# julius-speech/julius

Hardware: AMD Instinct MI355X
Metric: frames_x_states_scored_per_sec (higher is better)
Workload: dtype f32; 1 GPU; C2 = configs[1]: triphone GMM outprob only, S=3000 M=16 D=39, step = 12 launches x 64000 frames; frames_per_launch=64000, parallelism=utterance-sharded x1, kernel=gmm_tile<D=39,FPL=2,NS=16,ring> grid=24000 nsb=16

## Files before the change

julius_amd/csrc/gmm_outprob.hip:

```cpp
#include "gmm_dev.h"
#include "gmm_host.h"

namespace {
using namespace jamd;

constexpr int kWaves = 4;

template <int D, int FPL, int NS, bool HAS_NULL>
__global__ void __launch_bounds__(64 * kWaves)
gmm_tile_kernel(const float *__restrict__ rec, const int *__restrict__ st_off,
                const float *__restrict__ frames, const float *__restrict__ tbl,
                float *__restrict__ out, int T, int S, int nsb, int nfb, int nstb,
                float addmin_f) {
  static_assert(FPL % 2 == 0, "frames are processed as packed pairs");
  constexpr int REC = ((2 * D + 2) + 3) & ~3;
  constexpr int FPW = 64 * FPL;
  constexpr int NP = FPL / 2;
  __shared__ float tile[kWaves][FPW][NS + 1];

  int fb, sb;
  if (!decode_block(nfb, nstb, fb, sb)) return;
  const int lane = threadIdx.x & 63;
  const int wave = threadIdx.x >> 6;
  const int t0 = (fb * kWaves + wave) * FPW;
  if (t0 >= T) return;

  f2 v[NP][D];
#pragma unroll
  for (int p = 0; p < NP; p++) load_frames<D>(v[p], nullptr, frames, t0 + p * 128, T, D, lane);

#if defined(__HIP_DEVICE_COMPILE__) && !defined(__GFX9__)
#error "gmm_tile: the raw buffer descriptor below is the gfx9 (CDNA) format; this library is written for gfx950 only"
#endif
  const __amdgpu_buffer_rsrc_t tbl_rsrc = __builtin_amdgcn_make_buffer_rsrc((void *)tbl, 0, 4 * (JAMD_TBLSIZE + 1), 0x00020000);
  const int s_begin = sb * nsb;
  const int s_end = min(S, s_begin + nsb);
  for (int sg = s_begin; sg < s_end; sg += NS) {
    const int ns = min(NS, s_end - sg);
    for (int si = 0; si < ns; si++) {
      const int e0 = st_off[sg + si], e1 = st_off[sg + si + 1];
      f2 y2[NP], tv2[NP];
#pragma unroll
      for (int p = 0; p < NP; p++) { y2[p] = f2{JAMD_LOG_ZERO, JAMD_LOG_ZERO}; tv2[p] = f2{0.0f, 0.0f}; }
      for (int e = e1 - 1; e >= e0; e--) {
        const float *__restrict__ r = rec + (size_t)e * REC;
        const float gc = r[2 * D], lw = r[2 * D + 1];
        f2 acc[NP];
#pragma unroll
        for (int p = 0; p < NP; p++) acc[p] = f2{gc, gc};
#pragma unroll
        for (int d = 0; d < D; d++) {
          const float mu = r[d], iv = r[D + d];
          const f2 mu2 = {mu, mu}, iv2 = {iv, iv};
#pragma unroll
          for (int p = 0; p < NP; p++) {
            f2 x = v[p][d] - mu2;
            x = x * x;
            x = x * iv2;
            acc[p] = acc[p] + x;
          }
        }
        const bool nulld = HAS_NULL && (gc != gc);
        const float naddmin = -addmin_f;
#pragma unroll
        for (int p = 0; p < NP; p++) {
          f2 s2 = acc[p] * f2{-0.5f, -0.5f};
          if (nulld) s2 = f2{JAMD_LOG_ZERO, JAMD_LOG_ZERO};
          s2 = s2 + f2{lw, lw};
          __builtin_amdgcn_sched_barrier(0);
          const f2 yy = y2[p] + tv2[p];
          const f2 hi = {__builtin_fmaxf(s2.x, yy.x), __builtin_fmaxf(s2.y, yy.y)};
          const f2 df = s2 - yy;
          const float a0 = __builtin_fabsf(df.x), a1 = __builtin_fabsf(df.y);
          unsigned o0 = ((unsigned)((double)a0 * JAMD_TMAG + 0.5)) << 2, o1 = ((unsigned)((double)a1 * JAMD_TMAG + 0.5)) << 2;
          o0 = (a0 <= naddmin) ? o0 : 4u * (unsigned)JAMD_TBLSIZE;
          o1 = (a1 <= naddmin) ? o1 : 4u * (unsigned)JAMD_TBLSIZE;
          tv2[p] = f2{__builtin_bit_cast(float, __builtin_amdgcn_raw_buffer_load_b32(tbl_rsrc, (int)o0, 0, 0)),
                      __builtin_bit_cast(float, __builtin_amdgcn_raw_buffer_load_b32(tbl_rsrc, (int)o1, 0, 0))};
          y2[p] = hi;
        }
      }
#pragma unroll
      for (int k = 0; k < FPL; k++) {
        const f2 fin = y2[k / 2] + tv2[k / 2];
        tile[wave][k * 64 + lane][si] = finish_state((k & 1) ? fin.y : fin.x);
      }
    }
    wave_sync();
    constexpr int RPI = 64 / NS;
    const int col = lane % NS, rsub = lane / NS;
#pragma unroll 4
    for (int it = 0; it < FPW / RPI; it++) {
      const int rr = it * RPI + rsub;
      const int t = t0 + rr;
      if (t < T && col < ns) out[(size_t)t * S + sg + col] = tile[wave][rr][col];
    }
    wave_release();
  }
}

typedef float f16v __attribute__((ext_vector_type(16)));
constexpr int kRingRec = 80;

template <int BYTE_OFF>
__device__ __forceinline__ void ring_load(f16v &home, const float *chunks) {
  __builtin_amdgcn_sched_barrier(0);
  asm volatile("s_load_dwordx16 %0, %1, %2" : "=s"(home) : "s"(chunks), "i"(BYTE_OFF));
  __builtin_amdgcn_sched_barrier(0);
}
__device__ __forceinline__ void ring_wait(f16v &h0, f16v &h1, f16v &h2) {
  __builtin_amdgcn_sched_barrier(0);
  asm volatile("s_waitcnt lgkmcnt(0)" : "+s"(h0), "+s"(h1), "+s"(h2));
  __builtin_amdgcn_sched_barrier(0);
}
template <int N, int MU0, int IV0>
__device__ __forceinline__ void ring_chunk(f2 &acc, const f2 *v, const f16v &h) {
  f2 x[N], q[N], w[N];
#pragma unroll
  for (int i = 0; i < N + 3; i++) {
    if (i < N) { const float mu = h[MU0 + i]; x[i] = v[i] - f2{mu, mu}; }
    if (i >= 1 && i - 1 < N) q[i - 1] = x[i - 1] * x[i - 1];
    if (i >= 2 && i - 2 < N) { const float iv = h[IV0 + i - 2]; w[i - 2] = q[i - 2] * f2{iv, iv}; }
    if (i >= 3) acc = acc + w[i - 3];
    __builtin_amdgcn_sched_barrier(0);
  }
}

template <int NS, bool HAS_NULL>
__global__ void __launch_bounds__(64 * kWaves)
gmm_tile_ring_kernel(const float *__restrict__ ring, const int *__restrict__ st_off,
                     const float *__restrict__ frames, const float *__restrict__ tbl,
                     float *__restrict__ out, int T, int S, int nsb, int nfb, int nstb,
                     float addmin_f) {
  constexpr int D = 39, FPL = 2;
  constexpr int FPW = 64 * FPL;
  __shared__ float tile[kWaves][FPW][NS + 1];

  int fb, sb;
  if (!decode_block(nfb, nstb, fb, sb)) return;
  const int lane = threadIdx.x & 63;
  const int wave = threadIdx.x >> 6;
  const int t0 = (fb * kWaves + wave) * FPW;
  if (t0 >= T) return;

  f2 v[D];
  load_frames<D>(v, nullptr, frames, t0, T, D, lane);

  const __amdgpu_buffer_rsrc_t tbl_rsrc = __builtin_amdgcn_make_buffer_rsrc((void *)tbl, 0, 4 * (JAMD_TBLSIZE + 1), 0x00020000);
  const float naddmin = -addmin_f;
  const int s_begin = sb * nsb;
  const int s_end = min(S, s_begin + nsb);
  f16v h0, h1, h2;
  int held = -1;
  for (int sg = s_begin; sg < s_end; sg += NS) {
    const int ns = min(NS, s_end - sg);
    for (int si = 0; si < ns; si++) {
      const int s = sg + si;
      const int e0 = st_off[s], e1 = st_off[s + 1];
      const int e_over = (s + 1 < s_end ? st_off[s + 2] : e1) - 1;
      f2 y2 = {JAMD_LOG_ZERO, JAMD_LOG_ZERO}, tv2 = {0.0f, 0.0f};
      if (e1 > e0 && held != e1 - 1) {
        const float *r = ring + (size_t)(e1 - 1) * kRingRec;
        ring_load<0>(h0, r);
        ring_load<64>(h1, r);
        ring_load<128>(h2, r);
        ring_wait(h0, h1, h2);
      }
      for (int e = e1 - 1; e >= e0; e--) {
        const float *r = ring + (size_t)e * kRingRec;
        const float *rn = ring + (size_t)(e > e0 ? e - 1 : e_over) * kRingRec;
        const float gc = h0[0], lw = h0[1];
        const bool nulld = HAS_NULL && (gc != gc);
        f2 acc = {gc, gc};
        ring_chunk<7, 2, 9>(acc, v, h0);
        ring_load<192>(h0, r);
        ring_chunk<8, 0, 8>(acc, v + 7, h1);
        ring_load<256>(h1, r);
        ring_chunk<8, 0, 8>(acc, v + 15, h2);
        ring_wait(h0, h1, h2);
        ring_chunk<8, 0, 8>(acc, v + 23, h0);
        ring_load<0>(h0, rn);
        ring_load<128>(h2, rn);
        ring_chunk<8, 0, 8>(acc, v + 31, h1);
        ring_load<64>(h1, rn);
        {
          f2 s2 = acc * f2{-0.5f, -0.5f};
          if (nulld) s2 = f2{JAMD_LOG_ZERO, JAMD_LOG_ZERO};
          s2 = s2 + f2{lw, lw};
          __builtin_amdgcn_sched_barrier(0);
          const f2 yy = y2 + tv2;
          const f2 hi = {__builtin_fmaxf(s2.x, yy.x), __builtin_fmaxf(s2.y, yy.y)};
          const f2 df = s2 - yy;
          const float a0 = __builtin_fabsf(df.x), a1 = __builtin_fabsf(df.y);
          unsigned o0 = ((unsigned)((double)a0 * JAMD_TMAG + 0.5)) << 2, o1 = ((unsigned)((double)a1 * JAMD_TMAG + 0.5)) << 2;
          o0 = (a0 <= naddmin) ? o0 : 4u * (unsigned)JAMD_TBLSIZE;
          o1 = (a1 <= naddmin) ? o1 : 4u * (unsigned)JAMD_TBLSIZE;
          tv2 = f2{__builtin_bit_cast(float, __builtin_amdgcn_raw_buffer_load_b32(tbl_rsrc, (int)o0, 0, 0)),
                   __builtin_bit_cast(float, __builtin_amdgcn_raw_buffer_load_b32(tbl_rsrc, (int)o1, 0, 0))};
          y2 = hi;
        }
        ring_wait(h0, h1, h2);
      }
      if (e1 > e0) held = e_over;
      const f2 fin = y2 + tv2;
      tile[wave][lane][si] = finish_state(fin.x);
      tile[wave][64 + lane][si] = finish_state(fin.y);
    }
    store_tile<NS, FPW>(tile[wave], out, t0, T, S, sg, ns, lane);
  }
}

template <int FPL, int NS>
__global__ void __launch_bounds__(64 * kWaves)
gmm_tile_generic_kernel(const float *__restrict__ rec, const int *__restrict__ st_off,
                        const float *__restrict__ frames, const float *__restrict__ tbl,
                        float *__restrict__ out, int T, int S, int D, int REC, int nsb, int nfb,
                        int nstb, float addmin_f) {
  static_assert(FPL == 2, "load_frames / gauss_pair hold one packed pair of frames per lane");
  constexpr int FPW = 64 * FPL;
  __shared__ float tile[kWaves][FPW][NS + 1];
  extern __shared__ __align__(16) float dyn[];

  int fb, sb;
  if (!decode_block(nfb, nstb, fb, sb)) return;
  const int lane = threadIdx.x & 63;
  const int wave = threadIdx.x >> 6;
  const int t0 = (fb * kWaves + wave) * FPW;
  if (t0 >= T) return;
  float *vt = dyn + (size_t)wave * D * FPW;
  load_frames<0>(nullptr, vt, frames, t0, T, D, lane);

  const int s_begin = sb * nsb;
  const int s_end = min(S, s_begin + nsb);
  for (int sg = s_begin; sg < s_end; sg += NS) {
    const int ns = min(NS, s_end - sg);
    for (int si = 0; si < ns; si++) {
      const int e0 = st_off[sg + si], e1 = st_off[sg + si + 1];
      float y0 = JAMD_LOG_ZERO, y1 = JAMD_LOG_ZERO;
      for (int e = e1 - 1; e >= e0; e--) {
        const float *__restrict__ r = rec + (size_t)e * REC;
        const float lw = r[2 * D + 1];
        const f2 g = gauss_pair<0>(nullptr, vt, lane, D, r);
        y0 = addlog_step(y0, g.x + lw, tbl, addmin_f);
        y1 = addlog_step(y1, g.y + lw, tbl, addmin_f);
      }
      tile[wave][lane][si] = finish_state(y0);
      tile[wave][64 + lane][si] = finish_state(y1);
    }
    store_tile<NS, FPW>(tile[wave], out, t0, T, S, sg, ns, lane);
  }
}

template <int D, int FPL, int NS>
int launch_tile(jamd_gmm *g, const float *frames, int T, float *out, hipStream_t st) {
  constexpr int FPB = kWaves * 64 * FPL;
  const int nfb = (T + FPB - 1) / FPB;
  const int nsb = NS;
  const int nstb = (g->S + nsb - 1) / nsb;
  const int grid = xcd_grid(nstb, nfb);
  if constexpr (D == 39 && FPL == 2) {
    if (g->has_null)
      hipLaunchKernelGGL((gmm_tile_ring_kernel<NS, true>), dim3(grid), dim3(64 * kWaves), 0, st,
                         g->d_rec_ring, g->d_st_off_plain, frames, g->eng->d_addlog, out, T, g->S, nsb, nfb,
                         nstb, g->eng->addmin_f);
    else
      hipLaunchKernelGGL((gmm_tile_ring_kernel<NS, false>), dim3(grid), dim3(64 * kWaves), 0, st,
                         g->d_rec_ring, g->d_st_off_plain, frames, g->eng->d_addlog, out, T, g->S, nsb, nfb,
                         nstb, g->eng->addmin_f);
    snprintf(g->last_kernel, sizeof(g->last_kernel), "gmm_tile<D=%d,FPL=%d,NS=%d,ring> grid=%d nsb=%d", D, FPL, NS, grid, nsb);
  } else {
    if (g->has_null)
      hipLaunchKernelGGL((gmm_tile_kernel<D, FPL, NS, true>), dim3(grid), dim3(64 * kWaves), 0, st,
                         g->d_rec, g->d_st_off_plain, frames, g->eng->d_addlog, out, T, g->S, nsb, nfb,
                         nstb, g->eng->addmin_f);
    else
      hipLaunchKernelGGL((gmm_tile_kernel<D, FPL, NS, false>), dim3(grid), dim3(64 * kWaves), 0, st,
                         g->d_rec, g->d_st_off_plain, frames, g->eng->d_addlog, out, T, g->S, nsb, nfb,
                         nstb, g->eng->addmin_f);
    snprintf(g->last_kernel, sizeof(g->last_kernel), "gmm_tile<D=%d,FPL=%d,NS=%d> grid=%d nsb=%d", D, FPL, NS, grid, nsb);
  }
  return JAMD_OK;
}

template <int FPL, int NS>
int launch_tile_generic(jamd_gmm *g, const float *frames, int T, float *out, hipStream_t st) {
  constexpr int FPB = kWaves * 64 * FPL;
  const int nfb = (T + FPB - 1) / FPB;
  const int nsb = NS;
  const int nstb = (g->S + nsb - 1) / nsb;
  const int grid = xcd_grid(nstb, nfb);
  const size_t dyn = sizeof(float) * kWaves * g->D * 64 * FPL;
  const int rc = jamd_reserve_dyn_lds((const void *)gmm_tile_generic_kernel<FPL, NS>, dyn, "GMM outprob");
  if (rc != JAMD_OK) return rc;
  hipLaunchKernelGGL((gmm_tile_generic_kernel<FPL, NS>), dim3(grid), dim3(64 * kWaves), dyn, st,
                     g->d_rec, g->d_st_off_plain, frames, g->eng->d_addlog, out, T, g->S, g->D, g->rec,
                     nsb, nfb, nstb, g->eng->addmin_f);
  snprintf(g->last_kernel, sizeof(g->last_kernel), "gmm_tile_generic<FPL=%d,NS=%d> D=%d grid=%d",
           FPL, NS, g->D, grid);
  return JAMD_OK;
}

constexpr int kNarrowT = 256;
constexpr int kNarrowFB = 8;
template <int D, bool HAS_NULL>
__global__ void __launch_bounds__(64)
gmm_narrow_dens_kernel(const float *__restrict__ rec, const float *__restrict__ frames, float *__restrict__ dens, int T, int E,
                       int nfb, int neb) {
  constexpr int REC = (2 * D + 2 + 3) & ~3;
  int fbk, ebk;
  if (!decode_block(nfb, neb, fbk, ebk)) return;
  const int e = ebk * 64 + threadIdx.x;
  const float4 *__restrict__ r4 = reinterpret_cast<const float4 *>(rec + (size_t)(e < E ? e : E - 1) * REC);
  float r[REC];
#pragma unroll
  for (int q = 0; q < REC / 4; q++) { const float4 v = r4[q]; r[4 * q] = v.x; r[4 * q + 1] = v.y; r[4 * q + 2] = v.z; r[4 * q + 3] = v.w; }
  const float gc = r[2 * D], lw = r[2 * D + 1];
  const bool nulld = HAS_NULL && (gc != gc);
  const int t_end = min(T, (fbk + 1) * kNarrowFB);
  for (int t = fbk * kNarrowFB; t < t_end; t += 2) {
    const float *__restrict__ fa = frames + (size_t)t * D;
    const float *__restrict__ fb = frames + (size_t)(t + 1 < T ? t + 1 : t) * D;
    f2 acc = {gc, gc};
#pragma unroll
    for (int d = 0; d < D; d++) {
      f2 x = f2{fa[d], fb[d]} - f2{r[d], r[d]};
      x = x * x;
      x = x * f2{r[D + d], r[D + d]};
      acc = acc + x;
    }
    f2 s2 = acc * f2{-0.5f, -0.5f};
    if (nulld) s2 = f2{JAMD_LOG_ZERO, JAMD_LOG_ZERO};
    s2 = s2 + f2{lw, lw};
    if (e < E) {
      dens[(size_t)t * E + e] = s2.x;
      if (t + 1 < T) dens[(size_t)(t + 1) * E + e] = s2.y;
    }
  }
}

__global__ void __launch_bounds__(256)
gmm_narrow_lse_kernel(const float *__restrict__ dens, const int *__restrict__ st_off, const float *__restrict__ tbl,
                      float *__restrict__ out, int T, int S, int E, float addmin_f) {
  const int i = blockIdx.x * 256 + threadIdx.x;
  if (i >= T * S) return;
  const int t = i / S, s = i - t * S;
  const int e0 = st_off[s], e1 = st_off[s + 1];
  const float *__restrict__ dr = dens + (size_t)t * E;
  float y = JAMD_LOG_ZERO;
  int e = e1 - 1;
  for (; e - 7 >= e0; e -= 8) {
    float v[8];
#pragma unroll
    for (int q = 0; q < 8; q++) v[q] = dr[e - q];
#pragma unroll
    for (int q = 0; q < 8; q++) y = addlog_step(y, v[q], tbl, addmin_f);
  }
  for (; e >= e0; e--) y = addlog_step(y, dr[e], tbl, addmin_f);
  out[(size_t)t * S + s] = finish_state(y);
}

template <int D>
int launch_narrow(jamd_gmm *g, const float *frames, int T, float *out, hipStream_t st) {
  const int E = g->E_plain;
  int rc = jamd_grow(&g->d_narrow, &g->narrow_cap, sizeof(float) * (size_t)kNarrowT * (size_t)E);
  if (rc != JAMD_OK) return rc;
  const int grid = (E + 63) / 64;
  const int nfb = (T + kNarrowFB - 1) / kNarrowFB;
  const dim3 gr(xcd_grid(grid, nfb));
  if (g->has_null) hipLaunchKernelGGL((gmm_narrow_dens_kernel<D, true>), gr, dim3(64), 0, st, g->d_rec, frames, g->d_narrow, T, E, nfb, grid);
  else hipLaunchKernelGGL((gmm_narrow_dens_kernel<D, false>), gr, dim3(64), 0, st, g->d_rec, frames, g->d_narrow, T, E, nfb, grid);
  hipLaunchKernelGGL(gmm_narrow_lse_kernel, dim3((T * g->S + 255) / 256), dim3(256), 0, st, g->d_narrow, g->d_st_off_plain,
                     g->eng->d_addlog, out, T, g->S, E, g->eng->addmin_f);
  snprintf(g->last_kernel, sizeof(g->last_kernel), "gmm_narrow<D=%d> grid=%d + lse", D, grid);
  return JAMD_OK;
}

constexpr int kDensChunk = 1024;
__global__ void __launch_bounds__(64)
gmm_dens_kernel(const float *__restrict__ rec, const float *__restrict__ frames, float *__restrict__ out,
                int T, int E, int D, int REC) {
  extern __shared__ float xs[];
  float (*tile)[17] = reinterpret_cast<float (*)[17]>(xs + (size_t)D * 64);
  const int lane = threadIdx.x;
  const int t0 = blockIdx.x * 64, e_begin = blockIdx.y * kDensChunk;
  const int e_end = min(E, e_begin + kDensChunk);
  {
    int t = t0 + lane; if (t > T - 1) t = T - 1;
    const float *f = frames + (size_t)t * D;
    for (int d = 0; d < D; d++) xs[d * 64 + lane] = f[d];
  }
  wave_sync();
  for (int e0 = e_begin; e0 < e_end; e0 += 16) {
    const int ne = min(16, e_end - e0);
    for (int g = 0; g < ne; g++) {
      const float *__restrict__ r = rec + (size_t)(e0 + g) * REC;
      const float gc = r[2 * D];
      float acc = gc;
      for (int d = 0; d < D; d++) {
        float x = xs[d * 64 + lane] - r[d];
        x = x * x;
        x = x * r[D + d];
        acc = acc + x;
      }
      float sc = acc * -0.5f;
      if (gc != gc) sc = JAMD_LOG_ZERO;
      tile[lane][g] = sc;
    }
    wave_sync();
    const int col = lane & 15, rsub = lane >> 4;
    for (int it = 0; it < 16; it++) {
      const int rr = it * 4 + rsub, t = t0 + rr;
      if (t < T && col < ne) out[(size_t)t * E + e0 + col] = tile[rr][col];
    }
    wave_release();
  }
}

}


int jamd_gmm_launch_plain(jamd_gmm *g, const float *frames, int T, float *out, hipStream_t st) {
  const bool narrow = T <= kNarrowT && g->E_plain > 0;
  return dispatch_veclen(g->D, [&](auto dt) {
    constexpr int D = decltype(dt)::value;
    if constexpr (D == 0) return launch_tile_generic<2, 16>(g, frames, T, out, st);
    else return narrow ? launch_narrow<D>(g, frames, T, out, st) : launch_tile<D, 2, 16>(g, frames, T, out, st);
  });
}

int jamd_gmm_launch_dens(jamd_gmm *g, const float *rec, int E, const float *frames, int T, float *out, hipStream_t st) {
  const size_t lds = sizeof(float) * ((size_t)g->D * 64 + 64 * 17);
  if (lds > 64 * 1024) { jamd_set_error("jamd_gmm_dens_dev: vector length %d too large", g->D); return JAMD_EINVAL; }
  hipLaunchKernelGGL(gmm_dens_kernel, dim3((T + 63) / 64, (E + kDensChunk - 1) / kDensChunk), dim3(64), lds, st,
                     rec, frames, out, T, E, g->D, g->rec);
  return JAMD_OK;
}
```

julius_amd/csrc/engine.hip:

```cpp
#include "jamd_internal.h"
#include <cmath>
#include <mutex>

static thread_local char g_err[512] = "";

void jamd_set_error(const char *fmt, ...) {
  va_list ap;
  va_start(ap, fmt);
  vsnprintf(g_err, sizeof(g_err), fmt, ap);
  va_end(ap);
}

extern "C" {

int jamd_abi_version(void) { return JAMD_ABI_VERSION; }
const char *jamd_last_error(void) { return g_err; }

int jamd_device_count(void) {
  int n = 0;
  if (hipGetDeviceCount(&n) != hipSuccess) return 0;
  return n;
}

int jamd_engine_create(int device, jamd_engine **out) {
  if (!out) { jamd_set_error("jamd_engine_create: out is NULL"); return JAMD_EINVAL; }
  *out = nullptr;
  static std::once_flag queues_once;
  std::call_once(queues_once, [] { if (!getenv("GPU_MAX_HW_QUEUES")) setenv("GPU_MAX_HW_QUEUES", "16", 0); });
  int n = 0;
  hipError_t err = hipGetDeviceCount(&n);
  if (err != hipSuccess || n <= 0) {
    jamd_set_error("jamd_engine_create: no HIP device available (%s)",
                   err == hipSuccess ? "count is 0" : hipGetErrorString(err));
    return JAMD_ENODEV;
  }
  if (device < 0 || device >= n) {
    jamd_set_error("jamd_engine_create: device %d out of range [0,%d)", device, n);
    return JAMD_EINVAL;
  }
  JAMD_HIP(hipSetDevice(device));
  hipDeviceProp_t prop;
  JAMD_HIP(hipGetDeviceProperties(&prop, device));
  if (strncmp(prop.gcnArchName, "gfx950", 6) != 0) {
    jamd_set_error("jamd_engine_create: device %d is %s; this engine is built for gfx950 only",
                   device, prop.gcnArchName);
    return JAMD_ENODEV;
  }
  jamd_engine *e = new jamd_engine();
  e->device = device;
  e->num_cu = prop.multiProcessorCount;
  JAMD_HIP(hipStreamCreateWithFlags(&e->stream, hipStreamNonBlocking));

  std::vector<float> tbl(JAMD_TBLSIZE + 1);
  tbl[JAMD_TBLSIZE] = 0.0f;
  for (int i = 0; i < JAMD_TBLSIZE; i++) {
    float f = -((float)15 * (float)i / (float)JAMD_TBLSIZE);
    tbl[i] = (float)log(1 + exp(f));
  }
  JAMD_HIP(hipMalloc(&e->d_addlog, sizeof(float) * (JAMD_TBLSIZE + 1)));
  JAMD_HIP(hipMemcpy(e->d_addlog, tbl.data(), sizeof(float) * (JAMD_TBLSIZE + 1), hipMemcpyHostToDevice));
  std::vector<float> sig(JAMD_LOGISTIC_MAX + 1);
  for (int i = 0; i <= JAMD_LOGISTIC_MAX; i++) {
    double x = (double)i / (double)JAMD_LOGISTIC_FACTOR - 8.0;
    sig[i] = (float)(1.0 / (1.0 + exp(-x)));
  }
  JAMD_HIP(hipMalloc(&e->d_logistic, sizeof(float) * (JAMD_LOGISTIC_MAX + 1)));
  JAMD_HIP(hipMemcpy(e->d_logistic, sig.data(), sizeof(float) * (JAMD_LOGISTIC_MAX + 1),
                     hipMemcpyHostToDevice));
  float th = (float)JAMD_LOG_ADDMIN;
  if ((double)th < JAMD_LOG_ADDMIN) th = nextafterf(th, INFINITY);
  e->addmin_f = th;
  *out = e;
  return JAMD_OK;
}

void jamd_engine_destroy(jamd_engine *e) {
  if (!e) return;
  (void)hipSetDevice(e->device);
  if (e->d_addlog) (void)hipFree(e->d_addlog);
  if (e->d_logistic) (void)hipFree(e->d_logistic);
  if (e->stream) (void)hipStreamDestroy(e->stream);
  delete e;
}

int jamd_engine_device(const jamd_engine *e) { return e ? e->device : -1; }

int jamd_engine_sync(jamd_engine *e) {
  if (!e) { jamd_set_error("jamd_engine_sync: NULL engine"); return JAMD_EINVAL; }
  JAMD_HIP(hipSetDevice(e->device));
  JAMD_HIP(hipStreamSynchronize(e->stream));
  return JAMD_OK;
}

int jamd_malloc(jamd_engine *e, size_t bytes, void **dev) {
  if (!e || !dev) { jamd_set_error("jamd_malloc: NULL argument"); return JAMD_EINVAL; }
  JAMD_HIP(hipSetDevice(e->device));
  JAMD_HIP(hipMalloc(dev, bytes ? bytes : 4));
  return JAMD_OK;
}
int jamd_free(jamd_engine *e, void *dev) {
  if (!e) { jamd_set_error("jamd_free: NULL engine"); return JAMD_EINVAL; }
  JAMD_HIP(hipSetDevice(e->device));
  if (dev) JAMD_HIP(hipFree(dev));
  return JAMD_OK;
}
int jamd_host_alloc(jamd_engine *e, size_t bytes, void **host) {
  if (!e || !host) { jamd_set_error("jamd_host_alloc: NULL argument"); return JAMD_EINVAL; }
  JAMD_HIP(hipSetDevice(e->device));
  JAMD_HIP(hipHostMalloc(host, bytes ? bytes : 4, hipHostMallocDefault));
  return JAMD_OK;
}
int jamd_host_free(jamd_engine *e, void *host) {
  if (!e) { jamd_set_error("jamd_host_free: NULL engine"); return JAMD_EINVAL; }
  JAMD_HIP(hipSetDevice(e->device));
  if (host) JAMD_HIP(hipHostFree(host));
  return JAMD_OK;
}
int jamd_memcpy_h2d(jamd_engine *e, void *dev, const void *host, size_t bytes) {
  if (!e) { jamd_set_error("jamd_memcpy_h2d: NULL engine"); return JAMD_EINVAL; }
  JAMD_HIP(hipSetDevice(e->device));
  JAMD_HIP(hipMemcpyAsync(dev, host, bytes, hipMemcpyHostToDevice, e->stream));
  JAMD_HIP(hipStreamSynchronize(e->stream));
  return JAMD_OK;
}
int jamd_stream_create(jamd_engine *e, void **stream) {
  if (!e || !stream) { jamd_set_error("jamd_stream_create: NULL argument"); return JAMD_EINVAL; }
  JAMD_HIP(hipSetDevice(e->device));
  hipStream_t st = nullptr;
  JAMD_HIP(hipStreamCreateWithFlags(&st, hipStreamNonBlocking));
  *stream = (void *)st;
  return JAMD_OK;
}
int jamd_stream_destroy(jamd_engine *e, void *stream) {
  if (!e) { jamd_set_error("jamd_stream_destroy: NULL engine"); return JAMD_EINVAL; }
  JAMD_HIP(hipSetDevice(e->device));
  if (stream) JAMD_HIP(hipStreamDestroy((hipStream_t)stream));
  return JAMD_OK;
}
int jamd_stream_wait(jamd_engine *e, void *waiter, void *signaler) {
  if (!e) { jamd_set_error("jamd_stream_wait: NULL engine"); return JAMD_EINVAL; }
  JAMD_HIP(hipSetDevice(e->device));
  hipEvent_t ev = nullptr;
  JAMD_HIP(hipEventCreateWithFlags(&ev, hipEventDisableTiming));
  hipError_t rc = hipEventRecord(ev, jamd_stream(e, signaler));
  if (rc == hipSuccess) rc = hipStreamWaitEvent(jamd_stream(e, waiter), ev, 0);
  (void)hipEventDestroy(ev);
  if (rc != hipSuccess) { jamd_set_error("jamd_stream_wait: %s", hipGetErrorString(rc)); return JAMD_ENODEV; }
  return JAMD_OK;
}
int jamd_stream_sync(jamd_engine *e, void *stream) {
  if (!e) { jamd_set_error("jamd_stream_sync: NULL engine"); return JAMD_EINVAL; }
  JAMD_HIP(hipSetDevice(e->device));
  JAMD_HIP(hipStreamSynchronize(jamd_stream(e, stream)));
  return JAMD_OK;
}
int jamd_memcpy_h2d_async(jamd_engine *e, void *dev, const void *host, size_t bytes, void *stream) {
  if (!e) { jamd_set_error("jamd_memcpy_h2d_async: NULL engine"); return JAMD_EINVAL; }
  JAMD_HIP(hipSetDevice(e->device));
  JAMD_HIP(hipMemcpyAsync(dev, host, bytes, hipMemcpyHostToDevice, jamd_stream(e, stream)));
  return JAMD_OK;
}
int jamd_memcpy_d2h(jamd_engine *e, void *host, const void *dev, size_t bytes) {
  if (!e) { jamd_set_error("jamd_memcpy_d2h: NULL engine"); return JAMD_EINVAL; }
  JAMD_HIP(hipSetDevice(e->device));
  JAMD_HIP(hipMemcpyAsync(host, dev, bytes, hipMemcpyDeviceToHost, e->stream));
  JAMD_HIP(hipStreamSynchronize(e->stream));
  return JAMD_OK;
}

}
```

julius_amd/csrc/jamd_device.h:

```cpp
#pragma once
#include "jamd_internal.h"

namespace jamd {

__device__ __forceinline__ void wave_release() {
  __builtin_amdgcn_fence(__ATOMIC_RELEASE, "wavefront");
  __builtin_amdgcn_wave_barrier();
}
__device__ __forceinline__ void wave_sync() {
  wave_release();
  __builtin_amdgcn_fence(__ATOMIC_ACQUIRE, "wavefront");
}

__device__ __forceinline__ float addlog_step(float y, float sc, const float *__restrict__ tbl,
                                             float addmin_f) {
  const bool gt = sc > y;
  const float hi = gt ? sc : y;
  const float lo = gt ? y : sc;
  const float d = lo - hi;
  float r = hi;
  if (!(d < addmin_f)) {
    const unsigned idx = (unsigned)((double)(-d) * JAMD_TMAG + 0.5);
    r = hi + tbl[idx];
  }
  return r;
}

__device__ __forceinline__ float finish_state(float lse) {
  if (lse <= JAMD_LOG_ZERO || lse == 0.0f) return JAMD_LOG_ZERO;
  return (float)((double)lse * JAMD_INV_LOG_TEN);
}

constexpr int kNbestMax = 16;
template <typename Row>
__device__ __forceinline__ float cd_reduce(const Row &row, const int *__restrict__ states,
                                           int a, int b, int method, int nbest) {
  if (method == JAMD_IWCD_MAX) {
    float m = JAMD_LOG_ZERO;
    for (int k = a; k < b; k++) { const float p = row[states[k]]; if (m < p) m = p; }
    return m;
  }
  if (method == JAMD_IWCD_AVG) {
    float sum = 0.0f; int j = 0;
    for (int k = a; k < b; k++) { const float p = row[states[k]]; if (p > JAMD_LOG_ZERO) { sum += p; j++; } }
    return sum / (float)j;
  }
  if (nbest <= 4) {
    float b0 = JAMD_LOG_ZERO, b1 = JAMD_LOG_ZERO, b2 = JAMD_LOG_ZERO, b3 = JAMD_LOG_ZERO;
    int n = 0;
    auto ins = [&](float p) {
      if (p <= JAMD_LOG_ZERO) return;
      n++;
      float t;
      if (p > b0) { t = b0; b0 = p; p = t; }
      if (p > b1) { t = b1; b1 = p; p = t; }
      if (p > b2) { t = b2; b2 = p; p = t; }
      if (p > b3) { b3 = p; }
    };
    int k = a;
    for (; k + 4 <= b; k += 4) {
      const int s0 = states[k], s1 = states[k + 1], s2 = states[k + 2], s3 = states[k + 3];
      const float p0 = row[s0], p1 = row[s1], p2 = row[s2], p3 = row[s3];
      ins(p0); ins(p1); ins(p2); ins(p3);
    }
    for (; k < b; k++) ins(row[states[k]]);
    if (n > nbest) n = nbest;
    float sum = 0.0f;
    if (n > 0) sum += b0;
    if (n > 1) sum += b1;
    if (n > 2) sum += b2;
    if (n > 3) sum += b3;
    return sum / (float)n;
  }
  float best[kNbestMax];
  int n = 0;
#pragma unroll
  for (int q = 0; q < kNbestMax; q++) best[q] = JAMD_LOG_ZERO;
  for (int k = a; k < b; k++) {
    const float p = row[states[k]];
    if (p <= JAMD_LOG_ZERO) continue;
    int pos = 0;
#pragma unroll
    for (int q = 0; q < kNbestMax; q++) pos += (q < n && best[q] >= p) ? 1 : 0;
    if (pos >= nbest) continue;
#pragma unroll
    for (int q = kNbestMax - 1; q >= 1; q--) if (q > pos && q < nbest) best[q] = best[q - 1];
#pragma unroll
    for (int q = 0; q < kNbestMax; q++) if (q == pos) best[q] = p;
    if (n < nbest) n++;
  }
  float sum = 0.0f;
#pragma unroll
  for (int q = 0; q < kNbestMax; q++) if (q < n) sum += best[q];
  return sum / (float)n;
}

}
```

Measured before the change: 20.13 billion frame*states/s.

## Software-pipeline the whole 39-dim ring loop and use packed SGPR-operand math

Replaces the per-chunk software pipeline with a single continuous pipeline across all 39 dimensions, so the fill and drain stages no longer restart at every 8-element chunk boundary. Scalar-load refills for the next mixture are placed right after the last use of each 16-dword register block, so they are issued earlier. Subtract and multiply are written as inline v_pk_add/v_pk_mul asm that reads the mean and inverse variance as an SGPR pair through op_sel, which should avoid VGPR broadcast moves. The ring pointer is now advanced incrementally instead of being recomputed each iteration. The risks are the correctness of the hand-written op_sel encodings and the register-reuse timing for h2, which is now refilled before the h1 chunk.

```diff
diff --git a/julius_amd/csrc/gmm_outprob.hip b/julius_amd/csrc/gmm_outprob.hip
--- a/julius_amd/csrc/gmm_outprob.hip
+++ b/julius_amd/csrc/gmm_outprob.hip
@@ -113,16 +113,39 @@
   asm volatile("s_waitcnt lgkmcnt(0)" : "+s"(h0), "+s"(h1), "+s"(h2));
   __builtin_amdgcn_sched_barrier(0);
 }
-template <int N, int MU0, int IV0>
-__device__ __forceinline__ void ring_chunk(f2 &acc, const f2 *v, const f16v &h) {
-  f2 x[N], q[N], w[N];
-#pragma unroll
-  for (int i = 0; i < N + 3; i++) {
-    if (i < N) { const float mu = h[MU0 + i]; x[i] = v[i] - f2{mu, mu}; }
-    if (i >= 1 && i - 1 < N) q[i - 1] = x[i - 1] * x[i - 1];
-    if (i >= 2 && i - 2 < N) { const float iv = h[IV0 + i - 2]; w[i - 2] = q[i - 2] * f2{iv, iv}; }
-    if (i >= 3) acc = acc + w[i - 3];
+template <int K>
+__device__ __forceinline__ f2 ring_sub(const f2 a, const f16v &h) {
+  const f2 pr = __builtin_shufflevector(h, h, K & ~1, K | 1);
+  f2 r;
+  if constexpr (K & 1) asm("v_pk_add_f32 %0, %1, %2 op_sel:[0,1] op_sel_hi:[1,1] neg_lo:[0,1] neg_hi:[0,1]" : "=v"(r) : "v"(a), "s"(pr));
+  else asm("v_pk_add_f32 %0, %1, %2 op_sel_hi:[1,0] neg_lo:[0,1] neg_hi:[0,1]" : "=v"(r) : "v"(a), "s"(pr));
+  return r;
+}
+template <int K>
+__device__ __forceinline__ f2 ring_mul(const f2 a, const f16v &h) {
+  const f2 pr = __builtin_shufflevector(h, h, K & ~1, K | 1);
+  f2 r;
+  if constexpr (K & 1) asm("v_pk_mul_f32 %0, %1, %2 op_sel:[0,1] op_sel_hi:[1,1]" : "=v"(r) : "v"(a), "s"(pr));
+  else asm("v_pk_mul_f32 %0, %1, %2 op_sel_hi:[1,0]" : "=v"(r) : "v"(a), "s"(pr));
+  return r;
+}
+constexpr int ring_home(int d) { return d < 7 ? 0 : ((d - 7) / 8 + 1) % 3; }
+constexpr int ring_mu(int d) { return d < 7 ? 2 + d : (d - 7) % 8; }
+constexpr int ring_iv(int d) { return d < 7 ? 9 + d : 8 + (d - 7) % 8; }
+template <int H>
+__device__ __forceinline__ const f16v &ring_pick(const f16v &h0, const f16v &h1, const f16v &h2) {
+  if constexpr (H == 0) return h0; else if constexpr (H == 1) return h1; else return h2;
+}
+template <int A, int B>
+__device__ __forceinline__ void ring_steps(f2 &acc, const f2 *v, f2 *x, f2 *q, f2 *w, const f16v &h0, const f16v &h1, const f16v &h2) {
+  if constexpr (A < B) {
+    constexpr int D = 39;
+    if constexpr (A < D) x[A] = ring_sub<ring_mu(A)>(v[A], ring_pick<ring_home(A)>(h0, h1, h2));
+    if constexpr (A >= 1 && A - 1 < D) q[A - 1] = x[A - 1] * x[A - 1];
+    if constexpr (A >= 2 && A - 2 < D) w[A - 2] = ring_mul<ring_iv(A - 2)>(q[A - 2], ring_pick<ring_home(A - 2)>(h0, h1, h2));
+    if constexpr (A >= 3) acc = acc + w[A - 3];
     __builtin_amdgcn_sched_barrier(0);
+    ring_steps<A + 1, B>(acc, v, x, q, w, h0, h1, h2);
   }
 }
 
@@ -159,30 +182,35 @@
       const int e0 = st_off[s], e1 = st_off[s + 1];
       const int e_over = (s + 1 < s_end ? st_off[s + 2] : e1) - 1;
       f2 y2 = {JAMD_LOG_ZERO, JAMD_LOG_ZERO}, tv2 = {0.0f, 0.0f};
+      const float *r = ring + (ptrdiff_t)(e1 - 1) * kRingRec;
+      const float *r_over = ring + (ptrdiff_t)e_over * kRingRec;
       if (e1 > e0 && held != e1 - 1) {
-        const float *r = ring + (size_t)(e1 - 1) * kRingRec;
         ring_load<0>(h0, r);
         ring_load<64>(h1, r);
         ring_load<128>(h2, r);
         ring_wait(h0, h1, h2);
       }
       for (int e = e1 - 1; e >= e0; e--) {
-        const float *r = ring + (size_t)e * kRingRec;
-        const float *rn = ring + (size_t)(e > e0 ? e - 1 : e_over) * kRingRec;
-        const float gc = h0[0], lw = h0[1];
+        const float *rn = e > e0 ? r - kRingRec : r_over;
+        f2 gl;
+        asm("s_mov_b64 %0, %1" : "=s"(gl) : "s"(__builtin_shufflevector(h0, h0, 0, 1)));
+        const float gc = gl.x, lw = gl.y;
         const bool nulld = HAS_NULL && (gc != gc);
         f2 acc = {gc, gc};
-        ring_chunk<7, 2, 9>(acc, v, h0);
+        f2 x[D], q[D], w[D];
+        ring_steps<0, 9>(acc, v, x, q, w, h0, h1, h2);
         ring_load<192>(h0, r);
-        ring_chunk<8, 0, 8>(acc, v + 7, h1);
+        ring_steps<9, 17>(acc, v, x, q, w, h0, h1, h2);
         ring_load<256>(h1, r);
-        ring_chunk<8, 0, 8>(acc, v + 15, h2);
+        ring_steps<17, 23>(acc, v, x, q, w, h0, h1, h2);
         ring_wait(h0, h1, h2);
-        ring_chunk<8, 0, 8>(acc, v + 23, h0);
+        ring_steps<23, 25>(acc, v, x, q, w, h0, h1, h2);
+        ring_load<128>(h2, rn);
+        ring_steps<25, 33>(acc, v, x, q, w, h0, h1, h2);
         ring_load<0>(h0, rn);
-        ring_load<128>(h2, rn);
-        ring_chunk<8, 0, 8>(acc, v + 31, h1);
+        ring_steps<33, 42>(acc, v, x, q, w, h0, h1, h2);
         ring_load<64>(h1, rn);
+        r = rn;
         {
           f2 s2 = acc * f2{-0.5f, -0.5f};
           if (nulld) s2 = f2{JAMD_LOG_ZERO, JAMD_LOG_ZERO};
```

Measured after the change: 20.05 billion frame*states/s (median of 2 runs). Within noise of the previous version (-0.4%).

## Defer addlog table gather to next mixture iteration to overlap with distance compute

Applied to the files above, without the earlier changes.

The log-add table lookup for each mixture component is no longer issued right after its index is computed. The index is carried forward and the buffer load is issued at the top of the next iteration, before the Mahalanobis distance work, so that memory latency overlaps with arithmetic. The raw buffer descriptor is built by hand and the loads use inline asm with explicit waitcnt. The double-precision index computation becomes a single fused multiply-add, with a host helper that checks it matches the reference rounding. Risks are hand-rolled descriptor correctness, fma rounding differences, and an extra gather at the end of each state.

```diff
diff --git a/julius_amd/csrc/addlog_index.h b/julius_amd/csrc/addlog_index.h
--- /dev/null
+++ b/julius_amd/csrc/addlog_index.h
@@ -0,0 +1,45 @@
+#pragma once
+#include <cmath>
+#include <cstdint>
+#include <cstring>
+#include <vector>
+
+namespace jamd_addlog {
+
+constexpr int kTblSize = 500000;
+constexpr double kTmag = 33333.3333;
+constexpr double kLogAddMin = -13.815510558;
+
+inline uint32_t f2u(float f) { uint32_t u; std::memcpy(&u, &f, 4); return u; }
+inline float u2f(uint32_t u) { float f; std::memcpy(&f, &u, 4); return f; }
+
+inline std::vector<float> make_table() {
+  std::vector<float> tbl(kTblSize + 1);
+  for (int i = 0; i < kTblSize; i++) {
+    float f = -((float)15 * (float)i / (float)kTblSize);
+    tbl[i] = (float)log(1 + exp(f));
+  }
+  tbl[kTblSize] = 0.0f;
+  return tbl;
+}
+
+inline float addmin_float() {
+  float th = (float)kLogAddMin;
+  if ((double)th < kLogAddMin) th = nextafterf(th, INFINITY);
+  return th;
+}
+inline float cut() { return -addmin_float(); }
+
+inline unsigned ref_index(float a) {
+  volatile double p = (double)a * kTmag;
+  return (unsigned)(p + 0.5);
+}
+inline unsigned fma_index(float a) { return (unsigned)__builtin_fma((double)a, kTmag, 0.5); }
+
+inline long verify_range(uint32_t from, uint32_t to) {
+  long bad = 0;
+  for (uint32_t b = from; b < to; b++) bad += fma_index(u2f(b)) != ref_index(u2f(b));
+  return bad;
+}
+
+}
diff --git a/julius_amd/csrc/engine.hip b/julius_amd/csrc/engine.hip
--- a/julius_amd/csrc/engine.hip
+++ b/julius_amd/csrc/engine.hip
@@ -1,4 +1,5 @@
 #include "jamd_internal.h"
+#include "addlog_index.h"
 #include <cmath>
 #include <mutex>
 
@@ -51,12 +52,9 @@
   e->num_cu = prop.multiProcessorCount;
   JAMD_HIP(hipStreamCreateWithFlags(&e->stream, hipStreamNonBlocking));
 
-  std::vector<float> tbl(JAMD_TBLSIZE + 1);
-  tbl[JAMD_TBLSIZE] = 0.0f;
-  for (int i = 0; i < JAMD_TBLSIZE; i++) {
-    float f = -((float)15 * (float)i / (float)JAMD_TBLSIZE);
-    tbl[i] = (float)log(1 + exp(f));
-  }
+  static_assert(jamd_addlog::kTblSize == JAMD_TBLSIZE && jamd_addlog::kTmag == JAMD_TMAG && jamd_addlog::kLogAddMin == JAMD_LOG_ADDMIN,
+                "addlog_index.h restates the constants of jamd_internal.h");
+  const std::vector<float> tbl = jamd_addlog::make_table();
   JAMD_HIP(hipMalloc(&e->d_addlog, sizeof(float) * (JAMD_TBLSIZE + 1)));
   JAMD_HIP(hipMemcpy(e->d_addlog, tbl.data(), sizeof(float) * (JAMD_TBLSIZE + 1), hipMemcpyHostToDevice));
   std::vector<float> sig(JAMD_LOGISTIC_MAX + 1);
@@ -67,9 +65,7 @@
   JAMD_HIP(hipMalloc(&e->d_logistic, sizeof(float) * (JAMD_LOGISTIC_MAX + 1)));
   JAMD_HIP(hipMemcpy(e->d_logistic, sig.data(), sizeof(float) * (JAMD_LOGISTIC_MAX + 1),
                      hipMemcpyHostToDevice));
-  float th = (float)JAMD_LOG_ADDMIN;
-  if ((double)th < JAMD_LOG_ADDMIN) th = nextafterf(th, INFINITY);
-  e->addmin_f = th;
+  e->addmin_f = jamd_addlog::addmin_float();
   *out = e;
   return JAMD_OK;
 }
diff --git a/julius_amd/csrc/gmm_outprob.hip b/julius_amd/csrc/gmm_outprob.hip
--- a/julius_amd/csrc/gmm_outprob.hip
+++ b/julius_amd/csrc/gmm_outprob.hip
@@ -5,6 +5,28 @@
 using namespace jamd;
 
 constexpr int kWaves = 4;
+
+typedef unsigned u4v __attribute__((ext_vector_type(4)));
+#if defined(__HIP_DEVICE_COMPILE__) && !defined(__GFX9__)
+#error "gmm_tile: the buffer descriptor below is the gfx9 (CDNA) format; this library is written for gfx950 only"
+#endif
+__device__ __forceinline__ u4v table_rsrc(const float *tbl) {
+  const unsigned long long p = (unsigned long long)tbl;
+  return u4v{(unsigned)p, ((unsigned)(p >> 32) & 0xffffu) | (4u << 16), (unsigned)JAMD_TBLSIZE + 1u, 0x00020000u};
+}
+constexpr unsigned kNoTerm = JAMD_TBLSIZE;
+__device__ __forceinline__ void gather_issue(float &t, unsigned idx, const u4v &rs) {
+  asm volatile("buffer_load_dword %0, %1, %2, 0 idxen" : "=v"(t) : "v"(idx), "s"(rs));
+}
+__device__ __forceinline__ void logsum_index(unsigned &i0, unsigned &i1, f2 df, float naddmin) {
+  const float a0 = __builtin_fabsf(df.x), a1 = __builtin_fabsf(df.y);
+  i0 = (unsigned)__builtin_fma((double)a0, JAMD_TMAG, 0.5); i1 = (unsigned)__builtin_fma((double)a1, JAMD_TMAG, 0.5);
+  i0 = (a0 <= naddmin) ? i0 : kNoTerm;
+  i1 = (a1 <= naddmin) ? i1 : kNoTerm;
+}
+__device__ __forceinline__ void gather_wait(float &t0, float &t1) {
+  asm volatile("s_waitcnt vmcnt(0)" : "+v"(t0), "+v"(t1));
+}
 
 template <int D, int FPL, int NS, bool HAS_NULL>
 __global__ void __launch_bounds__(64 * kWaves)
@@ -29,20 +51,23 @@
 #pragma unroll
   for (int p = 0; p < NP; p++) load_frames<D>(v[p], nullptr, frames, t0 + p * 128, T, D, lane);
 
-#if defined(__HIP_DEVICE_COMPILE__) && !defined(__GFX9__)
-#error "gmm_tile: the raw buffer descriptor below is the gfx9 (CDNA) format; this library is written for gfx950 only"
-#endif
-  const __amdgpu_buffer_rsrc_t tbl_rsrc = __builtin_amdgcn_make_buffer_rsrc((void *)tbl, 0, 4 * (JAMD_TBLSIZE + 1), 0x00020000);
+  const u4v tbl_rsrc = table_rsrc(tbl);
   const int s_begin = sb * nsb;
   const int s_end = min(S, s_begin + nsb);
   for (int sg = s_begin; sg < s_end; sg += NS) {
     const int ns = min(NS, s_end - sg);
     for (int si = 0; si < ns; si++) {
       const int e0 = st_off[sg + si], e1 = st_off[sg + si + 1];
-      f2 y2[NP], tv2[NP];
-#pragma unroll
-      for (int p = 0; p < NP; p++) { y2[p] = f2{JAMD_LOG_ZERO, JAMD_LOG_ZERO}; tv2[p] = f2{0.0f, 0.0f}; }
+      f2 y2[NP];
+      unsigned ix[NP][2];
+      float tm[NP][2];
+#pragma unroll
+      for (int p = 0; p < NP; p++) { y2[p] = f2{JAMD_LOG_ZERO, JAMD_LOG_ZERO}; ix[p][0] = ix[p][1] = kNoTerm; }
       for (int e = e1 - 1; e >= e0; e--) {
+        __builtin_amdgcn_sched_barrier(0);
+#pragma unroll
+        for (int p = 0; p < NP; p++) { gather_issue(tm[p][0], ix[p][0], tbl_rsrc); gather_issue(tm[p][1], ix[p][1], tbl_rsrc); }
+        __builtin_amdgcn_sched_barrier(0);
         const float *__restrict__ r = rec + (size_t)e * REC;
         const float gc = r[2 * D], lw = r[2 * D + 1];
         f2 acc[NP];
@@ -68,18 +93,23 @@
           if (nulld) s2 = f2{JAMD_LOG_ZERO, JAMD_LOG_ZERO};
           s2 = s2 + f2{lw, lw};
           __builtin_amdgcn_sched_barrier(0);
-          const f2 yy = y2[p] + tv2[p];
+          gather_wait(tm[p][0], tm[p][1]);
+          __builtin_amdgcn_sched_barrier(0);
+          const f2 yy = y2[p] + f2{tm[p][0], tm[p][1]};
           const f2 hi = {__builtin_fmaxf(s2.x, yy.x), __builtin_fmaxf(s2.y, yy.y)};
-          const f2 df = s2 - yy;
-          const float a0 = __builtin_fabsf(df.x), a1 = __builtin_fabsf(df.y);
-          unsigned o0 = ((unsigned)((double)a0 * JAMD_TMAG + 0.5)) << 2, o1 = ((unsigned)((double)a1 * JAMD_TMAG + 0.5)) << 2;
-          o0 = (a0 <= naddmin) ? o0 : 4u * (unsigned)JAMD_TBLSIZE;
-          o1 = (a1 <= naddmin) ? o1 : 4u * (unsigned)JAMD_TBLSIZE;
-          tv2[p] = f2{__builtin_bit_cast(float, __builtin_amdgcn_raw_buffer_load_b32(tbl_rsrc, (int)o0, 0, 0)),
-                      __builtin_bit_cast(float, __builtin_amdgcn_raw_buffer_load_b32(tbl_rsrc, (int)o1, 0, 0))};
+          logsum_index(ix[p][0], ix[p][1], s2 - yy, naddmin);
           y2[p] = hi;
         }
       }
+      f2 tv2[NP];
+      __builtin_amdgcn_sched_barrier(0);
+#pragma unroll
+      for (int p = 0; p < NP; p++) {
+        gather_issue(tm[p][0], ix[p][0], tbl_rsrc); gather_issue(tm[p][1], ix[p][1], tbl_rsrc);
+        gather_wait(tm[p][0], tm[p][1]);
+        tv2[p] = f2{tm[p][0], tm[p][1]};
+      }
+      __builtin_amdgcn_sched_barrier(0);
 #pragma unroll
       for (int k = 0; k < FPL; k++) {
         const f2 fin = y2[k / 2] + tv2[k / 2];
@@ -146,7 +176,7 @@
   f2 v[D];
   load_frames<D>(v, nullptr, frames, t0, T, D, lane);
 
-  const __amdgpu_buffer_rsrc_t tbl_rsrc = __builtin_amdgcn_make_buffer_rsrc((void *)tbl, 0, 4 * (JAMD_TBLSIZE + 1), 0x00020000);
+  const u4v tbl_rsrc = table_rsrc(tbl);
   const float naddmin = -addmin_f;
   const int s_begin = sb * nsb;
   const int s_end = min(S, s_begin + nsb);
@@ -158,7 +188,9 @@
       const int s = sg + si;
       const int e0 = st_off[s], e1 = st_off[s + 1];
       const int e_over = (s + 1 < s_end ? st_off[s + 2] : e1) - 1;
-      f2 y2 = {JAMD_LOG_ZERO, JAMD_LOG_ZERO}, tv2 = {0.0f, 0.0f};
+      f2 y2 = {JAMD_LOG_ZERO, JAMD_LOG_ZERO};
+      unsigned ix0 = kNoTerm, ix1 = kNoTerm;
+      float tm0, tm1;
       if (e1 > e0 && held != e1 - 1) {
         const float *r = ring + (size_t)(e1 - 1) * kRingRec;
         ring_load<0>(h0, r);
@@ -172,6 +204,9 @@
         const float gc = h0[0], lw = h0[1];
         const bool nulld = HAS_NULL && (gc != gc);
         f2 acc = {gc, gc};
+        __builtin_amdgcn_sched_barrier(0);
+        gather_issue(tm0, ix0, tbl_rsrc);
+        gather_issue(tm1, ix1, tbl_rsrc);
         ring_chunk<7, 2, 9>(acc, v, h0);
         ring_load<192>(h0, r);
         ring_chunk<8, 0, 8>(acc, v + 7, h1);
@@ -188,21 +223,22 @@
           if (nulld) s2 = f2{JAMD_LOG_ZERO, JAMD_LOG_ZERO};
           s2 = s2 + f2{lw, lw};
           __builtin_amdgcn_sched_barrier(0);
-          const f2 yy = y2 + tv2;
+          gather_wait(tm0, tm1);
+          __builtin_amdgcn_sched_barrier(0);
+          const f2 yy = y2 + f2{tm0, tm1};
           const f2 hi = {__builtin_fmaxf(s2.x, yy.x), __builtin_fmaxf(s2.y, yy.y)};
-          const f2 df = s2 - yy;
-          const float a0 = __builtin_fabsf(df.x), a1 = __builtin_fabsf(df.y);
-          unsigned o0 = ((unsigned)((double)a0 * JAMD_TMAG + 0.5)) << 2, o1 = ((unsigned)((double)a1 * JAMD_TMAG + 0.5)) << 2;
-          o0 = (a0 <= naddmin) ? o0 : 4u * (unsigned)JAMD_TBLSIZE;
-          o1 = (a1 <= naddmin) ? o1 : 4u * (unsigned)JAMD_TBLSIZE;
-          tv2 = f2{__builtin_bit_cast(float, __builtin_amdgcn_raw_buffer_load_b32(tbl_rsrc, (int)o0, 0, 0)),
-                   __builtin_bit_cast(float, __builtin_amdgcn_raw_buffer_load_b32(tbl_rsrc, (int)o1, 0, 0))};
+          logsum_index(ix0, ix1, s2 - yy, naddmin);
           y2 = hi;
         }
         ring_wait(h0, h1, h2);
       }
       if (e1 > e0) held = e_over;
-      const f2 fin = y2 + tv2;
+      __builtin_amdgcn_sched_barrier(0);
+      gather_issue(tm0, ix0, tbl_rsrc);
+      gather_issue(tm1, ix1, tbl_rsrc);
+      gather_wait(tm0, tm1);
+      __builtin_amdgcn_sched_barrier(0);
+      const f2 fin = y2 + f2{tm0, tm1};
       tile[wave][lane][si] = finish_state(fin.x);
       tile[wave][64 + lane][si] = finish_state(fin.y);
     }
@@ -258,25 +294,17 @@
   const int nsb = NS;
   const int nstb = (g->S + nsb - 1) / nsb;
   const int grid = xcd_grid(nstb, nfb);
+  auto launch = [&](auto kernel, const float *records) {
+    hipLaunchKernelGGL(kernel, dim3(grid), dim3(64 * kWaves), 0, st, records, g->d_st_off_plain, frames, g->eng->d_addlog, out, T,
+                       g->S, nsb, nfb, nstb, g->eng->addmin_f);
+  };
   if constexpr (D == 39 && FPL == 2) {
-    if (g->has_null)
-      hipLaunchKernelGGL((gmm_tile_ring_kernel<NS, true>), dim3(grid), dim3(64 * kWaves), 0, st,
-                         g->d_rec_ring, g->d_st_off_plain, frames, g->eng->d_addlog, out, T, g->S, nsb, nfb,
-                         nstb, g->eng->addmin_f);
-    else
-      hipLaunchKernelGGL((gmm_tile_ring_kernel<NS, false>), dim3(grid), dim3(64 * kWaves), 0, st,
-                         g->d_rec_ring, g->d_st_off_plain, frames, g->eng->d_addlog, out, T, g->S, nsb, nfb,
-                         nstb, g->eng->addmin_f);
+    if (g->has_null) launch(gmm_tile_ring_kernel<NS, true>, g->d_rec_ring);
+    else launch(gmm_tile_ring_kernel<NS, false>, g->d_rec_ring);
     snprintf(g->last_kernel, sizeof(g->last_kernel), "gmm_tile<D=%d,FPL=%d,NS=%d,ring> grid=%d nsb=%d", D, FPL, NS, grid, nsb);
   } else {
-    if (g->has_null)
-      hipLaunchKernelGGL((gmm_tile_kernel<D, FPL, NS, true>), dim3(grid), dim3(64 * kWaves), 0, st,
-                         g->d_rec, g->d_st_off_plain, frames, g->eng->d_addlog, out, T, g->S, nsb, nfb,
-                         nstb, g->eng->addmin_f);
-    else
-      hipLaunchKernelGGL((gmm_tile_kernel<D, FPL, NS, false>), dim3(grid), dim3(64 * kWaves), 0, st,
-                         g->d_rec, g->d_st_off_plain, frames, g->eng->d_addlog, out, T, g->S, nsb, nfb,
-                         nstb, g->eng->addmin_f);
+    if (g->has_null) launch(gmm_tile_kernel<D, FPL, NS, true>, g->d_rec);
+    else launch(gmm_tile_kernel<D, FPL, NS, false>, g->d_rec);
     snprintf(g->last_kernel, sizeof(g->last_kernel), "gmm_tile<D=%d,FPL=%d,NS=%d> grid=%d nsb=%d", D, FPL, NS, grid, nsb);
   }
   return JAMD_OK;
diff --git a/julius_amd/csrc/jamd_device.h b/julius_amd/csrc/jamd_device.h
--- a/julius_amd/csrc/jamd_device.h
+++ b/julius_amd/csrc/jamd_device.h
@@ -20,7 +20,7 @@
   const float d = lo - hi;
   float r = hi;
   if (!(d < addmin_f)) {
-    const unsigned idx = (unsigned)((double)(-d) * JAMD_TMAG + 0.5);
+    const unsigned idx = (unsigned)__builtin_fma((double)(-d), JAMD_TMAG, 0.5);
     r = hi + tbl[idx];
   }
   return r;
```

Result: no change. 20.39 billion frame*states/s before, 20.39 billion frame*states/s after, median of 3 (+0.0%).
